# GeWu-Lab/Crab

Measured on AMD Instinct MI355X. Metric: clips/sec prefill+decode (AVQA 10s clip, 8 frames, 256 out tok), higher is better.
Workload: dtype bf16

## Files before the change

### crab_amd/_lib.py

```python
from __future__ import annotations

import ctypes as C
import os
import threading

_HERE = os.path.dirname(os.path.abspath(__file__))
LIB_PATH = os.environ.get("CRAB_HIP_LIB") or os.path.join(_HERE, "libcrab_hip.so")


class CrabHipError(RuntimeError):
    pass


class GemmDesc(C.Structure):
    _fields_ = [
        ("A", C.c_void_p), ("B", C.c_void_p), ("C", C.c_void_p), ("bias", C.c_void_p), ("R", C.c_void_p),
        ("A2", C.c_void_p), ("B2", C.c_void_p),
        ("lda", C.c_int64), ("ldb", C.c_int64), ("ldc", C.c_int64), ("ldr", C.c_int64), ("lda2", C.c_int64),
        ("ldb2", C.c_int64),
        ("M", C.c_int32), ("N", C.c_int32), ("K", C.c_int32), ("K2", C.c_int32),
        ("act", C.c_int32), ("c_fp32", C.c_int32), ("res_scale", C.c_float),
        ("batch", C.c_int32), ("nb0", C.c_int32),
        ("sA0", C.c_int64), ("sA1", C.c_int64), ("sB0", C.c_int64), ("sB1", C.c_int64), ("sC0", C.c_int64),
        ("sC1", C.c_int64), ("sR0", C.c_int64), ("sR1", C.c_int64), ("sBias0", C.c_int64), ("sBias1", C.c_int64),
# ... 123 lines not shown
    "crab_trace_end": (_i64, [_vp, C.c_char_p, _i64]),
    "crab_gemm_bf16": (_i, [_vp, _vp, C.POINTER(GemmDesc)]),
    "crab_rowfin_workspace": (_i64, [_i, _i]),
    "crab_rowfin_lora_ok": (_i, [_i, _i, _i]),
    "crab_attn_decode_rope_workspace": (_i64, [_i, _i, _i]),
    "crab_attn_decode_rope": (_i, [_vp, _vp, _vp, _i64, _vp, _vp, _vp, _vp, _i64, _i, _i, _i, _i, _i, _i, _vp, _f, _vp, _i64]),
    "crab_attn_prefix_workspace": (_i64, [_i, _i, _i]),
    "crab_attn_prefix_partial": (_i, [_vp, _vp, _vp, _i64, _vp, _vp, _vp, _i64, _vp, _i, _vp, _i, _i, _i, _i, _i, _i, _i, _f]),
    "crab_attn_own_merge": (_i, [_vp, _vp, _vp, _i64, _vp, _i64, _vp, _vp, _vp, _i64, _i, _i, _i, _i, _i, _i, _i, _vp, _f, _vp]),
    "crab_hyperlora_mix": (_i, [_vp, _vp, _vp, _i64, _i, _vp, _i64, _i, _i, _i, _i, _i, _f]),
    "crab_hyperlora_route_workspace": (_i64, [_i, _i, _i]),
    "crab_hyperlora_route": (_i, [_vp, _vp, _vp, _i64, _vp, _i64, _i, _i, _i, _i, _i, _vp, _i64, _i, _f, _vp, _i64]),
    "crab_rmsnorm": (_i, [_vp, _vp, _vp, _i64, _vp, _vp, _i64, _i, _i, _f]),
    "crab_layernorm": (_i, [_vp, _vp, _vp, _i64, _vp, _vp, _vp, _i64, _i, _i, _f]),
    "crab_embedding": (_i, [_vp, _vp, _vp, _vp, _vp, _i64, _i, _i, _i]),
    "crab_embedding_f32": (_i, [_vp, _vp, _vp, _vp, _vp, _i64, _i, _i, _i]),
    "crab_rmsnorm_f32": (_i, [_vp, _vp, _vp, _i64, _vp, _vp, _i64, _i, _i, _f]),
    "crab_layernorm_f32": (_i, [_vp, _vp, _vp, _i64, _vp, _vp, _vp, _i64, _i, _i, _f]),
    "crab_rmsnorm_p": (_i, [_vp, _vp, _vp, _i, _i64, _vp, _i, _vp, _i64, _i, _i, _f]),
    "crab_layernorm_p": (_i, [_vp, _vp, _vp, _i, _i64, _vp, _vp, _i, _vp, _i64, _i, _i, _f]),
    "crab_clip_embed_ln_p": (_i, [_vp, _vp, _vp, _vp, _vp, _vp, _vp, _i, _vp, _i, _i, _i, _f]),
    "crab_cast_rows_bf16_f32": (_i, [_vp, _vp, _vp, _i64, _vp, _i64, _i, _i]),
    "crab_cast_rows_f32_bf16": (_i, [_vp, _vp, _vp, _i64, _vp, _i64, _i, _i]),
    "crab_rope_table": (_i, [_vp, _vp, _vp, _i, _i, _f]),
    "crab_qkv_rope_split": (_i, [_vp, _vp, _vp, _i64, _vp, _vp, _vp, _vp, _i64, _i, _i, _i, _i, _i, _i, _i, _vp]),
    "crab_qkv_rope_split_ids": (_i, [_vp, _vp, _vp, _i64, _vp, _vp, _vp, _vp, _i64, _i, _i, _i, _i, _i, _i, _i, _vp, _vp, _i64]),
    "crab_qkv_rope_split_ragged": (_i, [_vp, _vp, _vp, _i64, _vp, _vp, _vp, _vp, _i64, _i, _i, _i, _i, _i, _i, _i, _vp, _vp]),
    "crab_kv_quant_fp8": (_i, [_vp, _vp, _vp, _vp, _i64, _i, _i, _vp, _vp, _i64, _vp, _vp, _i64, _i, _i, _i, _i, _i, _i, _i, _i, _vp]),
    "crab_weight_quant_fp8": (_i, [_vp, _vp, _vp, _i64, _i, _i, _vp, _i64, _vp]),
    "crab_attn_decode_fp8": (_i, [_vp, _vp, _vp, _i64, _vp, _vp, _vp, _vp, _vp, _vp, _i64, _i, _i, _i, _i, _i, _i, _vp, _f, _vp]),
    "crab_attn_decode_masked": (_i, [_vp, _vp, _vp, _i64, _vp, _vp, _vp, _i64, _i, _i, _i, _i, _i, _i, _vp, _f, _vp]),
    "crab_attn_decode_keymask": (_i, [_vp, _vp, _vp, _i64, _vp, _vp, _vp, _i64, _i, _i, _i, _i, _i, _i, _vp, _f, _vp, _i64]),
    "crab_attn_fwd": (_i, [_vp, _vp, C.POINTER(AttnDesc)]),
    "crab_attn_decode": (_i, [_vp, _vp, _vp, _i64, _vp, _vp, _vp, _i64, _i, _i, _i, _i, _i, _i, _vp, _f]),
    "crab_swiglu": (_i, [_vp, _vp, _vp, _i64, _vp, _i64, _i, _i]),
    "crab_argmax": (_i, [_vp, _vp, _vp, _i64, _vp, _i, _i, _i]),
    "crab_im2col_patch": (_i, [_vp, _vp, _vp, _i, _vp, _i64, _i, _i, _i, _i, _i]),
    "crab_clip_embed_ln": (_i, [_vp, _vp, _vp, _vp, _vp, _vp, _vp, _vp, _i, _i, _i, _f]),
    "crab_beats_posconv_pad": (_i, [_vp, _vp, _vp, _vp, _i, _i, _i, _i, _i]),
    "crab_beats_relpos_bias": (_i, [_vp, _vp, _vp, _vp, _i, _i, _i, _i]),
    "crab_beats_gru_gate": (_i, [_vp, _vp, _vp, _i64, _vp, _vp, _vp, _vp, _i, _i, _i, _i]),
    "crab_copy_rows": (_i, [_vp, _vp, _vp, _i64, _vp, _i64, _i, _i]),
    "crab_cast_f32_bf16": (_i, [_vp, _vp, _vp, _vp, _i64]),
    "crab_copy_rows_batched": (_i, [_vp, _vp, _vp, _i64, _i64, _vp, _i64, _i64, _i, _i, _i]),
    "crab_greedy_select": (_i, [_vp, _vp, _vp, _i64, _i, _i, _vp, _vp, _i64, _vp, _vp, _i, _i, _i]),
    "crab_advance": (_i, [_vp, _vp, _vp, _vp]),
    "crab_sample_select": (_i, [_vp, _vp, _vp, _i64, _i, _i, _vp, _vp, _i64, _vp, _vp, _i, _i, _i, _f, _i, _f, C.c_uint64]),
    "crab_constrained_select": (_i, [_vp, _vp, _vp, _i64, _i, _i, _vp, _vp, _vp, _i, _i, _vp, _vp, _vp, _i64, _vp, _vp, _i, _i, _i, _f, _i, _f,
                                     C.c_uint64]),
    "crab_logprob_norm": (_i, [_vp, _vp, _vp, _i64, _i, _i, _vp, _vp, _i, _i, _vp, _vp, _vp, _i, _i, _vp]),
    "crab_logprob_gather": (_i, [_vp, _vp, _vp, _i64, _i, _i, _vp, _vp, _vp, _vp, _i64, _i64, _i]),
    "crab_logits_edit": (_i, [_vp, _vp, _vp, _i64, _i, _i, _vp, _i64, _i, _vp, _vp, _f, _i, _vp, _i, _i, _vp, _vp, _i64]),
    "crab_logits_restore": (_i, [_vp, _vp, _vp, _i64, _i, _i, _vp, _vp, _vp, _i, _vp, _vp, _i64, _i]),
    "crab_lm_head_xent_workspace": (_i64, [_i, _i]),
    "crab_lm_head_xent": (_i, [_vp, _vp, _vp, _i64, _vp, _i, _vp, _i64, _i, _i, _vp, _vp, _vp, _vp, _vp, _i64]),
    "crab_xent_reduce": (_i, [_vp, _vp, _vp, _vp, _vp, _vp, _i, _vp, _vp, _vp, _vp]),
    "crab_im2col3x3": (_i, [_vp, _vp, _vp, _vp, _i, _i, _i, _i]),
    "crab_pixel_shuffle2x": (_i, [_vp, _vp, _vp, _vp, _vp, _i, _i, _i]),
    "crab_bilinear": (_i, [_vp, _vp, _vp, _i, _i64, _i64, _i64, _i, _i, _i, _vp, _i, _i, _f, _f]),
    "crab_dense_pe": (_i, [_vp, _vp, _vp, _vp, _i, _i, _i]),
    "crab_add_rows": (_i, [_vp, _vp, _vp, _i64, _vp, _i64, _i, _vp, _i64, _i, _i]),
    "crab_mask_gate": (_i, [_vp, _vp, _vp, _i64, _i, _vp, _i64, _i, _i]),
    "crab_act_inplace": (_i, [_vp, _vp, _vp, _i64, _i]),
    "crab_dist_unique_id": (_i, [_vp, _vp]),
    "crab_dist_init": (_i, [_vp, _vp, _i, _i, C.POINTER(_vp)]),
    "crab_gather_results": (_i, [_vp, _vp, _vp, _vp, _i64, _vp, _i]),
# ... 87 lines not shown
```

### crab_amd/csrc/attn.hip

```cpp
#include "common.h"
#include "crab_internal.h"
#include "attn_decode_core.h"
#include <math.h>
#include <stdlib.h>

namespace {

struct AttnP {
    const bf16_t* q; const bf16_t* k; const bf16_t* vt; bf16_t* o;
    long q_bs, q_hs, q_ss, k_bs, k_hs, k_ss, vt_bs, vt_hs, vt_ds, o_bs, o_ss;
    const float* bias; const float* gate;
    const int* kv_start;
    const uint32_t* key_mask; long key_mask_ld;
    int B, H, Hk, Sq, Skv, causal;
    float scale;
};

constexpr int KT = 64;
constexpr int VT_LD = 68;

template <int HD>
__device__ __forceinline__ int k_swz(int row, int chunk) {
    return HD == 128 ? (chunk ^ (row & 15)) : (HD == 64 ? (chunk ^ ((row >> 1) & 7)) : (chunk ^ ((0x78 >> (((row >> 2) & 3) * 2)) & 3)));
}
// ... 159 lines not shown
        for (int kk = 0; kk < 2; ++kk) {
            union { bf16x8_t v; uint32_t w[4]; } pf;
            pf.w[0] = pack_bf2(s[2 * kk][0], s[2 * kk][1]);
            pf.w[1] = pack_bf2(s[2 * kk][2], s[2 * kk][3]);
            pf.w[2] = pack_bf2(s[2 * kk + 1][0], s[2 * kk + 1][1]);
            pf.w[3] = pack_bf2(s[2 * kk + 1][2], s[2 * kk + 1][3]);
#pragma unroll
            for (int dt = 0; dt < DT; ++dt) {
                const bf16_t* vr = lv + (dt * 16 + fr) * VT_LD + kk * 32 + fg * 4;
                union { bf16x8_t v; u32x2 h[2]; } vf;
                vf.h[0] = *reinterpret_cast<const u32x2*>(vr);
                vf.h[1] = *reinterpret_cast<const u32x2*>(vr + 16);
                oacc[dt] = __builtin_amdgcn_mfma_f32_16x16x32_bf16(vf.v, pf.v, oacc[dt], 0, 0, 0);
            }
        }
    }
    l_run += __shfl_xor(l_run, 16, 64);
    l_run += __shfl_xor(l_run, 32, 64);
    const float inv = l_run > 0.f ? 1.0f / l_run : 0.f;
    if (qrow < p.Sq) {
        bf16_t* op = p.o + (long)b * p.o_bs + (long)qrow * p.o_ss + (long)h * HD;
#pragma unroll
        for (int dt = 0; dt < DT; ++dt) {
            u32x2 w;
            w[0] = pack_bf2(oacc[dt][0] * inv, oacc[dt][1] * inv);
            w[1] = pack_bf2(oacc[dt][2] * inv, oacc[dt][3] * inv);
            *reinterpret_cast<u32x2*>(op + dt * 16 + fg * 4) = w;
        }
    }
}


typedef __attribute__((ext_vector_type(16))) float f32x16_t;

template <int HD, bool CAUSAL>
__global__ __launch_bounds__(256, 2) void attn_fwd32_kernel(AttnP p) {
    constexpr int CPR = HD / 8;
    constexpr int KS = HD / 16;
    constexpr int DT = HD / 32;
    constexpr int KBUF = KT * HD, VBUF = HD * VT_LD;
    __shared__ __attribute__((aligned(16))) bf16_t lk[2 * KBUF];
    __shared__ __attribute__((aligned(16))) bf16_t lv[2 * VBUF];

    const int tid = threadIdx.x, lane = tid & 63;
    const int wave = __builtin_amdgcn_readfirstlane(tid >> 6);
    const int fc = lane & 31, fg = lane >> 5;
    const int nqb = (p.Sq + 127) >> 7;
    const int lid = xcd_remap(blockIdx.x, gridDim.x);
    const int b = lid / (nqb * p.H), h = (lid / nqb) % p.H;
    const int hk = h / (p.H / p.Hk);
    const int q0 = (nqb - 1 - lid % nqb) * 128;
    const int qw0 = q0 + wave * 32;
    const int qrow = qw0 + fc;
    const int qload = qrow < p.Sq ? qrow : p.Sq - 1;
    const int koff = p.Skv - p.Sq;
    const bool wave_on = qw0 < p.Sq;

    const bf16_t* qp = p.q + (long)b * p.q_bs + (long)h * p.q_hs + (long)qload * p.q_ss;
    const bf16_t* kp = p.k + (long)b * p.k_bs + (long)hk * p.k_hs;
    const bf16_t* vp = p.vt + (long)b * p.vt_bs + (long)hk * p.vt_hs;

    bf16x8_t qf[KS];
#pragma unroll
    for (int ks = 0; ks < KS; ++ks) qf[ks] = *reinterpret_cast<const bf16x8_t*>(qp + ks * 16 + fg * 8);

    f32x16_t oacc[DT];
// ... 98 lines not shown
                for (int r = 0; r < 16; ++r) {
                    const float e = __builtin_amdgcn_exp2f(__builtin_fmaf(s[j][r], sc2, -m_new));
                    s[j][r] = e;
                    psum += e;
                }
            l_run = l_run * alpha + psum;
            if (__any(raised)) {
#pragma unroll
                for (int i = 0; i < DT; ++i) oacc[i] *= alpha;
            }
#pragma unroll
            for (int j = 0; j < 2; ++j)
#pragma unroll
                for (int kk = 0; kk < 2; ++kk) {
                    union { bf16x8_t v; uint32_t w[4]; } pf;
                    pf.w[0] = pack_bf2(s[j][8 * kk + 0], s[j][8 * kk + 1]);
                    pf.w[1] = pack_bf2(s[j][8 * kk + 2], s[j][8 * kk + 3]);
                    pf.w[2] = pack_bf2(s[j][8 * kk + 4], s[j][8 * kk + 5]);
                    pf.w[3] = pack_bf2(s[j][8 * kk + 6], s[j][8 * kk + 7]);
#pragma unroll
                    for (int dt = 0; dt < DT; ++dt) {
                        const bf16_t* vr = lvc + (dt * 32 + fc) * VT_LD + j * 32 + kk * 16 + fg * 4;
                        union { bf16x8_t v; u32x2 hh[2]; } vf;
                        vf.hh[0] = *reinterpret_cast<const u32x2*>(vr);
                        vf.hh[1] = *reinterpret_cast<const u32x2*>(vr + 8);
                        oacc[dt] = __builtin_amdgcn_mfma_f32_32x32x16_bf16(vf.v, pf.v, oacc[dt], 0, 0, 0);
                    }
                }
        }
        __syncthreads();
    }
    l_run += __shfl_xor(l_run, 32, 64);
    const float inv = l_run > 0.f ? 1.0f / l_run : 0.f;
    if (qrow < p.Sq) {
        bf16_t* op = p.o + (long)b * p.o_bs + (long)qrow * p.o_ss + (long)h * HD;
#pragma unroll
        for (int dt = 0; dt < DT; ++dt)
#pragma unroll
            for (int g4 = 0; g4 < 4; ++g4) {
                u32x2 w;
                w[0] = pack_bf2(oacc[dt][4 * g4 + 0] * inv, oacc[dt][4 * g4 + 1] * inv);
                w[1] = pack_bf2(oacc[dt][4 * g4 + 2] * inv, oacc[dt][4 * g4 + 3] * inv);
                *reinterpret_cast<u32x2*>(op + dt * 32 + g4 * 8 + fg * 4) = w;
            }
    }
}
#undef ATT_LOAD_TILE
#undef ATT_MASK_V
#undef ATT_STORE_TILE

template <int HD>
__global__ __launch_bounds__(256) void attn_decode_kernel(const bf16_t* __restrict__ q, long ldq, const bf16_t* __restrict__ kc,
                                                          const bf16_t* __restrict__ vc, bf16_t* __restrict__ o, long ldo, int H, int Hk,
                                                          int Tmax, int ctx_host, const int* __restrict__ ctx_dev, float scale,
                                                          const int* __restrict__ kv_start) {
    constexpr int EPL = HD / 16;
    const int tid = threadIdx.x;
    const int grp = tid >> 4, sub = tid & 15;
    const int b = blockIdx.y, h = blockIdx.x;
    const int hk = h / (H / Hk);
    const int ks0 = kv_start ? kv_start[b] : 0;
    const int ctx = ctx_host + (ctx_dev ? ctx_dev[0] : 0) - ks0;
    const bf16_t* qp = q + (long)b * ldq + (long)h * HD + sub * EPL;
    float qv[EPL];
#pragma unroll
    for (int e = 0; e < EPL; ++e) qv[e] = bf2f(qp[e]) * scale;
    const bf16_t* kb = kc + (((long)b * Hk + hk) * (long)Tmax + ks0) * HD + sub * EPL;
    const bf16_t* vb = vc + (((long)b * Hk + hk) * (long)Tmax + ks0) * HD + sub * EPL;
    float m = -1e30f, l = 0.f, acc[EPL];
#pragma unroll
    for (int e = 0; e < EPL; ++e) acc[e] = 0.f;
    if constexpr (EPL == 8) {
        dec_stream(qv, kb, vb, ctx, grp, m, l, acc);
    } else {
        for (int j = grp; j < ctx; j += 16) {
            float kx[EPL], vx[EPL];
            const u32x2 kw = __builtin_nontemporal_load(reinterpret_cast<const u32x2*>(kb + (long)j * HD));
            const u32x2 vw = __builtin_nontemporal_load(reinterpret_cast<const u32x2*>(vb + (long)j * HD));
#pragma unroll
            for (int e = 0; e < 2; ++e) { kx[2 * e] = lo_bf(kw[e]); kx[2 * e + 1] = hi_bf(kw[e]); vx[2 * e] = lo_bf(vw[e]); vx[2 * e + 1] = hi_bf(vw[e]); }
            float sdot = 0.f;
#pragma unroll
// ... 382 lines not shown
#pragma unroll
                for (int g = 0; g < G; ++g) {
                    const float pg = g < 4 ? p0[g & 3] : p1[g & 3];
#pragma unroll
                    for (int e = 0; e < EPL; ++e) acc[g][e] += pg * vx[e];
                }
            }
        }
    }
    __syncthreads();
#pragma unroll
    for (int g = 0; g < G; ++g)
#pragma unroll
        for (int e = 0; e < EPL; ++e) {
            float v = acc[g][e];
            v += __shfl_xor(v, 16, 64);
            v += __shfl_xor(v, 32, 64);
            acc[g][e] = v;
        }
    if (lane < 16) {
#pragma unroll
        for (int g = 0; g < G; ++g)
#pragma unroll
            for (int e = 0; e < EPL; ++e) sbuf[(wave * G + g) * HD + sub * EPL + e] = acc[g][e];
    }
    __syncthreads();
    for (int idx = tid; idx < G * HD; idx += 256) {
        const float O = (sbuf[idx] + sbuf[G * HD + idx]) + (sbuf[2 * G * HD + idx] + sbuf[3 * G * HD + idx]);
        const int g = idx / HD;
        o[(long)b * ldo + (long)(hk * G) * HD + idx] = f2bf(O / l_run[g]);
    }
}

}

extern "C" int crab_attn_fwd(crab_ctx* ctx, void* stream, const crab_attn_desc* d) {
    if (!ctx) return CRAB_E_INVALID;
    if (!d || !d->q || !d->k || !d->vt || !d->o) return crab_fail(ctx, CRAB_E_INVALID, "attn_fwd: null operand");
    if (d->B <= 0 || d->H <= 0 || d->Hk <= 0 || d->H % d->Hk || d->Sq <= 0 || d->Skv <= 0)
        return crab_fail(ctx, CRAB_E_INVALID, "attn_fwd: bad shape");
    if (d->head_dim != 32 && d->head_dim != 64 && d->head_dim != 128) return crab_fail(ctx, CRAB_E_UNSUPPORTED, "attn_fwd: head_dim must be 32, 64 or 128");
    if (d->head_dim == 32 && (d->causal || d->bias)) return crab_fail(ctx, CRAB_E_UNSUPPORTED, "attn_fwd: head_dim 32 only without mask/bias");
    if ((d->q_ss & 7) || (d->q_hs & 7) || (d->q_bs & 7) || (d->k_ss & 7) || (d->k_hs & 7) || (d->k_bs & 7) || (d->vt_ds & 7) ||
        (d->vt_hs & 7) || (d->vt_bs & 7) || (d->o_ss & 3) || (d->o_bs & 3))
        return crab_fail(ctx, CRAB_E_INVALID, "attn_fwd: strides must keep 16-byte alignment");
    if (((uintptr_t)d->q & 15) || ((uintptr_t)d->k & 15) || ((uintptr_t)d->vt & 15) || ((uintptr_t)d->o & 7))
        return crab_fail(ctx, CRAB_E_INVALID, "attn_fwd: pointer alignment");
    if (d->causal && d->Skv < d->Sq) return crab_fail(ctx, CRAB_E_INVALID, "attn_fwd: causal needs Skv >= Sq");
    if ((d->bias == nullptr) && d->gate) return crab_fail(ctx, CRAB_E_INVALID, "attn_fwd: gate without bias");
    if (d->key_mask && (d->key_mask_ld < (d->Skv + 31) / 32 || d->head_dim == 32))
        return crab_fail(ctx, CRAB_E_INVALID, "attn_fwd: key_mask needs key_mask_ld >= ceil(Skv / 32) words per sequence (head_dim 64 / 128)");
    AttnP p;
    p.q = (const bf16_t*)d->q; p.k = (const bf16_t*)d->k; p.vt = (const bf16_t*)d->vt; p.o = (bf16_t*)d->o;
    p.q_bs = d->q_bs; p.q_hs = d->q_hs; p.q_ss = d->q_ss; p.k_bs = d->k_bs; p.k_hs = d->k_hs; p.k_ss = d->k_ss;
    p.vt_bs = d->vt_bs; p.vt_hs = d->vt_hs; p.vt_ds = d->vt_ds; p.o_bs = d->o_bs; p.o_ss = d->o_ss;
    p.bias = d->bias; p.gate = d->gate; p.kv_start = d->kv_start; p.key_mask = d->key_mask; p.key_mask_ld = d->key_mask_ld; p.B = d->B; p.H = d->H; p.Hk = d->Hk; p.Sq = d->Sq; p.Skv = d->Skv;
    p.causal = d->causal; p.scale = d->scale;
    dim3 grid(((d->Sq + 63) / 64) * d->H * d->B), block(256);
    hipStream_t s = (hipStream_t)stream;
    const bool hb = d->bias != nullptr;
    if (d->causal && hb) return crab_fail(ctx, CRAB_E_UNSUPPORTED, "attn_fwd: causal + bias not instantiated");
    static const int fwd32 = []() { const char* e = getenv("CRAB_ATTN_FWD32"); return !(e && e[0] == '0'); }();
    if (fwd32 && !hb && d->Sq > 64 && d->scale > 0.f && (d->head_dim == 128 || d->head_dim == 64)) {
        dim3 grid32(((d->Sq + 127) / 128) * d->H * d->B);
        if (d->head_dim == 128) {
            if (d->causal) hipLaunchKernelGGL((attn_fwd32_kernel<128, true>), grid32, block, 0, s, p);
            else hipLaunchKernelGGL((attn_fwd32_kernel<128, false>), grid32, block, 0, s, p);
        } else {
            if (d->causal) hipLaunchKernelGGL((attn_fwd32_kernel<64, true>), grid32, block, 0, s, p);
            else hipLaunchKernelGGL((attn_fwd32_kernel<64, false>), grid32, block, 0, s, p);
        }
        return crab_check_launch(ctx, d->head_dim == 128 ? (d->causal ? "attn_fwd32_kernel<128,causal>" : "attn_fwd32_kernel<128>")
                                                         : (d->causal ? "attn_fwd32_kernel<64,causal>" : "attn_fwd32_kernel<64>"));
    }
    if (d->head_dim == 32) {
        hipLaunchKernelGGL((attn_fwd_kernel<32, false, false>), grid, block, 0, s, p);
    } else if (d->head_dim == 128) {
        if (d->causal) hipLaunchKernelGGL((attn_fwd_kernel<128, true, false>), grid, block, 0, s, p);
        else if (hb) hipLaunchKernelGGL((attn_fwd_kernel<128, false, true>), grid, block, 0, s, p);
        else hipLaunchKernelGGL((attn_fwd_kernel<128, false, false>), grid, block, 0, s, p);
    } else {
        if (d->causal) hipLaunchKernelGGL((attn_fwd_kernel<64, true, false>), grid, block, 0, s, p);
        else if (hb) hipLaunchKernelGGL((attn_fwd_kernel<64, false, true>), grid, block, 0, s, p);
        else hipLaunchKernelGGL((attn_fwd_kernel<64, false, false>), grid, block, 0, s, p);
    }
    return crab_check_launch(ctx, d->head_dim == 32 ? "attn_fwd_kernel<32>" : d->head_dim == 128 ? (d->causal ? "attn_fwd_kernel<128,causal>" : hb ? "attn_fwd_kernel<128,bias>" : "attn_fwd_kernel<128>")
                                                                            : (d->causal ? "attn_fwd_kernel<64,causal>" : hb ? "attn_fwd_kernel<64,bias>" : "attn_fwd_kernel<64>"));
}

extern "C" int64_t crab_attn_decode_rope_workspace(int B, int H, int d) {
    return ((int64_t)B * H * 8 * (d + 2) * 4 + 255) / 256 * 256 + (int64_t)B * H * 4;
}

extern "C" int crab_attn_decode_rope(crab_ctx* ctx, void* stream, const void* qkv, int64_t ldqkv, const float* rope_tab, void* k_cache,
                                     void* v_cache, void* o, int64_t ldo, int B, int H, int Hk, int d, int Tmax, int pos0,
                                     const int32_t* pos_dev, float scale, void* workspace, int64_t workspace_bytes) {
    if (!ctx) return CRAB_E_INVALID;
    if (!qkv || !rope_tab || !k_cache || !v_cache || !o || B <= 0 || H <= 0 || Hk <= 0 || H % Hk) return crab_fail(ctx, CRAB_E_INVALID, "attn_decode_rope: bad argument");
    if (d != 64 && d != 128) return crab_fail(ctx, CRAB_E_UNSUPPORTED, "attn_decode_rope: head_dim must be 64 or 128");
    if ((ldqkv & 7) || ((uintptr_t)qkv & 15) || ((uintptr_t)k_cache & 15) || ((uintptr_t)v_cache & 15)) return crab_fail(ctx, CRAB_E_INVALID, "attn_decode_rope: alignment");
    if (!pos_dev && (pos0 < 0 || pos0 >= Tmax)) return crab_fail(ctx, CRAB_E_INVALID, "attn_decode_rope: position outside the KV cache");
    int nsplit = 1;
    static const int tgt = []() { const char* e = getenv("CRAB_ATTN_BLOCKS"); return e ? atoi(e) : 512; }();
    if ((long)B * H < tgt) { nsplit = (int)(tgt / ((long)B * H)); if (nsplit > 8) nsplit = 8; }
    if (nsplit > 1 && (!workspace || workspace_bytes < crab_attn_decode_rope_workspace(B, H, d)))
        return crab_fail(ctx, CRAB_E_WORKSPACE, "attn_decode_rope: needs crab_attn_decode_rope_workspace(B, H, d) bytes (counters zeroed once)");
    float* part = (float*)workspace;
    unsigned* counters = workspace ? (unsigned*)((char*)workspace + ((int64_t)B * H * 8 * (d + 2) * 4 + 255) / 256 * 256) : nullptr;
    hipStream_t s = (hipStream_t)stream;
    static const int wide_on = []() { const char* e = getenv("CRAB_ATTN_WIDE"); return !(e && e[0] == '0'); }();
    if (wide_on && nsplit == 2 && d == 128) {
        hipLaunchKernelGGL((attn_decode_rope_kernel<128, 32>), dim3(H, B, 1), dim3(512), 0, s, (const bf16_t*)qkv, (long)ldqkv, rope_tab, (bf16_t*)k_cache,
                           (bf16_t*)v_cache, (bf16_t*)o, (long)ldo, H, Hk, Tmax, pos0, pos_dev, scale, (float*)nullptr, (unsigned*)nullptr);
        return crab_check_launch(ctx, "attn_decode_rope_kernel<128,32>");
    }
    dim3 grid(H, B, nsplit), block(256);
    if (d == 128)
        hipLaunchKernelGGL((attn_decode_rope_kernel<128>), grid, block, 0, s, (const bf16_t*)qkv, (long)ldqkv, rope_tab, (bf16_t*)k_cache,
                           (bf16_t*)v_cache, (bf16_t*)o, (long)ldo, H, Hk, Tmax, pos0, pos_dev, scale, part, counters);
    else
// ... 59 lines not shown
```

### crab_amd/ops.py

```python
from __future__ import annotations

import ctypes as C
import os
from typing import Optional

import torch

from . import _lib
from ._lib import AttnDesc, GemmDesc

ACT = {"none": 0, None: 0, "gelu": 1, "quick_gelu": 2, "relu": 3, "silu": 4, "swiglu_pair": 5}
BF16 = torch.bfloat16


def _stream():
    return C.c_void_p(torch.cuda.current_stream().cuda_stream)


def _dev(t: torch.Tensor) -> int:
    if not t.is_cuda:
        raise _lib.CrabHipError("crab_amd ops need CUDA/HIP tensors (no CPU fallback exists)")
    return t.device.index or 0


# ... 307 lines not shown
        _lib.check(_lib.load().crab_cast_rows_f32_bf16(_lib.ctx(d), _stream(), _p(src), lds, _p(dst), dst.stride(0), rows, cols), d)
    else:
        raise _lib.CrabHipError(f"cast_rows: {src.dtype} -> {dst.dtype} is not supported")
    return dst


def rope_table(max_pos: int, head_dim: int, theta: float, device) -> torch.Tensor:
    tab = torch.empty((max_pos, head_dim // 2, 2), device=device, dtype=torch.float32)
    d = _dev(tab)
    _lib.check(_lib.load().crab_rope_table(_lib.ctx(d), _stream(), _p(tab), max_pos, head_dim, theta), d)
    return tab


def qkv_rope_split(qkv: torch.Tensor, rope_tab: Optional[torch.Tensor], k_cache: Optional[torch.Tensor],
                   v_cache: Optional[torch.Tensor], vt: Optional[torch.Tensor], B: int, S: int, H: int, Hk: int, d_: int,
                   Tmax: int, pos0: int = 0, pos_dev: Optional[torch.Tensor] = None, pos_ids: Optional[torch.Tensor] = None,
                   row_off: Optional[torch.Tensor] = None):
    d = _dev(qkv)
    vt_ld = vt.stride(-2) if vt is not None else 0
    if row_off is not None:
        if pos_ids is not None:
            raise ValueError("qkv_rope_split: pos_ids and row_off are alternatives")
        _lib.check(_lib.load().crab_qkv_rope_split_ragged(_lib.ctx(d), _stream(), _p(qkv), qkv.stride(0), _p(rope_tab), _p(k_cache), _p(v_cache),
                                                          _p(vt), vt_ld, B, S, H, Hk, d_, Tmax, pos0, _p(pos_dev), _p(row_off)), d)
        return
    if pos_ids is not None and (pos_ids.dtype != torch.int32 or pos_ids.dim() != 2 or pos_ids.stride(1) != 1):
        raise ValueError("pos_ids must be an int32 [B, S] tensor with contiguous rows")
    _lib.check(_lib.load().crab_qkv_rope_split_ids(_lib.ctx(d), _stream(), _p(qkv), qkv.stride(0), _p(rope_tab), _p(k_cache), _p(v_cache),
                                                   _p(vt), vt_ld, B, S, H, Hk, d_, Tmax, pos0, _p(pos_dev), _p(pos_ids),
                                                   pos_ids.stride(0) if pos_ids is not None else 0), d)


def attn_fwd(q, k, vt, o, *, q_strides, k_strides, vt_strides, o_strides, B, H, Hk, Sq, Skv, head_dim, scale, causal=False,
             bias=None, gate=None, kv_start=None, key_mask=None):
    d = _dev(q)
    a = AttnDesc()
    a.q, a.k, a.vt, a.o = q.data_ptr(), k.data_ptr(), vt.data_ptr(), o.data_ptr()
    a.q_bs, a.q_hs, a.q_ss = q_strides
    a.k_bs, a.k_hs, a.k_ss = k_strides
    a.vt_bs, a.vt_hs, a.vt_ds = vt_strides
    a.o_bs, a.o_ss = o_strides
    a.bias = bias.data_ptr() if bias is not None else None
    a.gate = gate.data_ptr() if gate is not None else None
    a.kv_start = kv_start.data_ptr() if kv_start is not None else None
    if key_mask is not None:
        if key_mask.dtype != torch.int32 or key_mask.dim() != 2 or key_mask.stride(1) != 1 or key_mask.shape[0] != B:
            raise ValueError("key_mask must be an int32 [B, words] tensor with contiguous rows (ops.pack_key_mask)")
        a.key_mask, a.key_mask_ld = key_mask.data_ptr(), key_mask.stride(0)
    a.B, a.H, a.Hk, a.Sq, a.Skv, a.head_dim, a.causal, a.scale = B, H, Hk, Sq, Skv, head_dim, 1 if causal else 0, scale
    _lib.check(_lib.load().crab_attn_fwd(_lib.ctx(d), _stream(), C.byref(a)), d)
    return o


def pack_key_mask(mask: torch.Tensor) -> torch.Tensor:
    m = mask.reshape(mask.shape[0], -1).ne(0)
    B, T = m.shape
    W = (T + 31) // 32
    mp = torch.zeros(B, W * 32, dtype=torch.int64, device=m.device)
    mp[:, :T] = m
    v = (mp.view(B, W, 32) << torch.arange(32, device=m.device)).sum(-1)
    return torch.where(v >= 2 ** 31, v - 2 ** 32, v).to(torch.int32).contiguous()


def attn_decode(q, k_cache, v_cache, o, B, H, Hk, head_dim, Tmax, ctx_len, scale, ctx_dev=None, kv_start=None, key_mask=None):
    d = _dev(q)
    if key_mask is not None:
        if kv_start is not None:
            raise ValueError("attn_decode: key_mask already carries the left padding, pass one of the two")
        if key_mask.dtype != torch.int32 or key_mask.dim() != 2 or key_mask.stride(1) != 1 or key_mask.shape[0] != B:
            raise ValueError("key_mask must be an int32 [B, words] tensor with contiguous rows (ops.pack_key_mask)")
        _lib.check(_lib.load().crab_attn_decode_keymask(_lib.ctx(d), _stream(), _p(q), q.stride(0), _p(k_cache), _p(v_cache), _p(o), o.stride(0),
                                                        B, H, Hk, head_dim, Tmax, ctx_len, _p(ctx_dev), scale, _p(key_mask), key_mask.stride(0)), d)
        return o
    prof = PROFILER
    sample = prof is not None and prof.decode_eager and prof.decode_ctx > 0 and not torch.cuda.is_current_stream_capturing()
    if sample:
        e0 = torch.cuda.Event(enable_timing=True); e1 = torch.cuda.Event(enable_timing=True)
        e0.record()
    _lib.check(_lib.load().crab_attn_decode_masked(_lib.ctx(d), _stream(), _p(q), q.stride(0), _p(k_cache), _p(v_cache), _p(o), o.stride(0),
                                                   B, H, Hk, head_dim, Tmax, ctx_len, _p(ctx_dev), scale, _p(kv_start)), d)
    if sample:
        e1.record()
        nbytes = 2.0 * B * prof.decode_ctx * Hk * head_dim * 2 + 2.0 * B * H * head_dim * 2
# ... 614 lines not shown
```

### include/crab_hip.h

```cpp
#ifndef CRAB_HIP_H
#define CRAB_HIP_H

#include <stdint.h>

#ifdef __cplusplus
extern "C" {
#endif

#define CRAB_OK 0
#define CRAB_E_INVALID (-1)
#define CRAB_E_HIP (-2)
#define CRAB_E_UNSUPPORTED (-3)
#define CRAB_E_WORKSPACE (-4)

typedef struct crab_ctx crab_ctx;

int crab_ctx_create(int device, crab_ctx** out);
void crab_ctx_destroy(crab_ctx* ctx);
const char* crab_last_error(crab_ctx* ctx);
int crab_sync(crab_ctx* ctx, void* stream);
int crab_abi_version(void);
int crab_trace_begin(crab_ctx* ctx);
int64_t crab_trace_end(crab_ctx* ctx, char* buf , int64_t n);
int crab_sizeof_gemm_desc(void);
// ... 61 lines not shown
int crab_rmsnorm_p(crab_ctx* ctx, void* stream, const void* x, int x_fp32, int64_t ldx, const void* w, int w_fp32, void* y, int64_t ldy,
                   int M, int D, float eps);

int crab_embedding(crab_ctx* ctx, void* stream, const int64_t* ids, const void* table, void* out, int64_t ldo,
                   int T, int D, int vocab);
int crab_embedding_f32(crab_ctx* ctx, void* stream, const int64_t* ids, const void* table, float* out, int64_t ldo,
                       int T, int D, int vocab);

int crab_rope_table(crab_ctx* ctx, void* stream, float* tab, int max_pos, int head_dim, float theta);

int crab_qkv_rope_split(crab_ctx* ctx, void* stream, void* qkv, int64_t ldqkv, const float* rope_tab,
                        void* k_cache, void* v_cache, void* vt, int64_t vt_ld, int B, int S, int H, int Hk, int d,
                        int Tmax, int pos0, const int32_t* pos_dev);

int crab_qkv_rope_split_ids(crab_ctx* ctx, void* stream, void* qkv, int64_t ldqkv, const float* rope_tab,
                            void* k_cache, void* v_cache, void* vt, int64_t vt_ld, int B, int S, int H, int Hk, int d,
                            int Tmax, int pos0, const int32_t* pos_dev, const int32_t* pos_ids, int64_t ld_pos);

int crab_qkv_rope_split_ragged(crab_ctx* ctx, void* stream, void* qkv, int64_t ldqkv, const float* rope_tab,
                               void* k_cache, void* v_cache, void* vt, int64_t vt_ld, int B, int S, int H, int Hk, int d,
                               int Tmax, int pos0, const int32_t* pos_dev, const int32_t* row_off);


typedef struct {
    const void* q; const void* k; const void* vt; void* o;
    int64_t q_bs, q_hs, q_ss, k_bs, k_hs, k_ss, vt_bs, vt_hs, vt_ds, o_bs, o_ss;
    const float* bias; const float* gate;
    int32_t B, H, Hk, Sq, Skv, head_dim, causal;
    float scale;
    const int32_t* kv_start;
    const uint32_t* key_mask; int64_t key_mask_ld;
} crab_attn_desc;
int crab_attn_fwd(crab_ctx* ctx, void* stream, const crab_attn_desc* d);

int crab_attn_decode(crab_ctx* ctx, void* stream, const void* q, int64_t ldq, const void* k_cache, const void* v_cache,
                     void* o, int64_t ldo, int B, int H, int Hk, int d, int Tmax, int ctx_len_host,
                     const int32_t* ctx_dev, float scale);

int crab_attn_decode_masked(crab_ctx* ctx, void* stream, const void* q, int64_t ldq, const void* k_cache, const void* v_cache,
                            void* o, int64_t ldo, int B, int H, int Hk, int d, int Tmax, int ctx_len_host,
                            const int32_t* ctx_dev, float scale, const int32_t* kv_start);
int crab_attn_decode_keymask(crab_ctx* ctx, void* stream, const void* q, int64_t ldq, const void* k_cache, const void* v_cache,
                             void* o, int64_t ldo, int B, int H, int Hk, int d, int Tmax, int ctx_len_host, const int32_t* ctx_dev,
                             float scale, const uint32_t* key_mask, int64_t key_mask_ld);

#define CRAB_ATTN_SPLIT_BELOW 257
int64_t crab_attn_decode_rope_workspace(int B, int H, int d);
int crab_attn_decode_rope(crab_ctx* ctx, void* stream, const void* qkv, int64_t ldqkv, const float* rope_tab, void* k_cache,
                          void* v_cache, void* o, int64_t ldo, int B, int H, int Hk, int d, int Tmax, int pos0,
                          const int32_t* pos_dev, float scale, void* workspace, int64_t workspace_bytes);

int64_t crab_attn_prefix_workspace(int rows, int H, int d);
int crab_attn_prefix_partial(crab_ctx* ctx, void* stream, const void* q, int64_t ldq, const void* prefix_k, const void* prefix_v,
                             void* workspace, int64_t workspace_bytes, const int32_t* tile_rows, int ntiles, const int32_t* row_clip,
                             int rows, int C, int H, int Hk, int d, int Tp, int P, float scale);
int crab_attn_own_merge(crab_ctx* ctx, void* stream, const void* q, int64_t ldq, const void* workspace, int64_t workspace_bytes,
                        const void* k_cache, const void* v_cache, void* o, int64_t ldo, int B, int Sq, int H, int Hk, int d, int Tmax,
                        int ctx_len_host, const int32_t* ctx_dev, float scale, const int32_t* kv_start);

int crab_kv_quant_fp8(crab_ctx* ctx, void* stream, const void* k_src, const void* v_src, int64_t src_layer_stride, int T_src, int t0,
                      void* k_codes, void* v_codes, int64_t code_layer_stride, float* k_scale, float* v_scale,
                      int64_t scale_layer_stride, int L, int Bc, int Hk, int d, int Tmax, int b0, int t_dst, int S,
                      const int32_t* row_off);
int crab_attn_decode_fp8(crab_ctx* ctx, void* stream, const void* qkv, int64_t ldqkv, const float* rope_tab, void* k_codes,
                         void* v_codes, float* k_scale, float* v_scale, void* o, int64_t ldo, int B, int H, int Hk, int d, int Tmax,
                         int pos0, const int32_t* pos_dev, float scale, const int32_t* kv_start);
// ... 189 lines not shown
```

Before: 30.96.

## Add 8-wave ping-pong attention forward kernel and wide permlane output stores

Adds an opt-in 512-thread attention prefill kernel in which two wave groups are staggered by one KV tile, so one group's QK/PV MFMA work can overlap the other's softmax and global-to-LDS loads. It is reachable only through a new form argument, since the automatic flags are off. The existing 4-wave kernel's epilogue is also changed to use permlane32 swaps, giving 16-byte output stores when the output pointer and strides are aligned. That store path runs by default and aims to cut store instruction count, at the cost of extra cross-lane swap operations.

```diff
diff --git a/crab_amd/_lib.py b/crab_amd/_lib.py
--- a/crab_amd/_lib.py
+++ b/crab_amd/_lib.py
@@ -179,6 +179,7 @@
     "crab_attn_decode_masked": (_i, [_vp, _vp, _vp, _i64, _vp, _vp, _vp, _i64, _i, _i, _i, _i, _i, _i, _vp, _f, _vp]),
     "crab_attn_decode_keymask": (_i, [_vp, _vp, _vp, _i64, _vp, _vp, _vp, _i64, _i, _i, _i, _i, _i, _i, _vp, _f, _vp, _i64]),
     "crab_attn_fwd": (_i, [_vp, _vp, C.POINTER(AttnDesc)]),
+    "crab_attn_fwd_form": (_i, [_vp, _vp, C.POINTER(AttnDesc), _i]),
     "crab_attn_decode": (_i, [_vp, _vp, _vp, _i64, _vp, _vp, _vp, _i64, _i, _i, _i, _i, _i, _i, _vp, _f]),
     "crab_swiglu": (_i, [_vp, _vp, _vp, _i64, _vp, _i64, _i, _i]),
     "crab_argmax": (_i, [_vp, _vp, _vp, _i64, _vp, _i, _i, _i]),
diff --git a/crab_amd/csrc/attn.hip b/crab_amd/csrc/attn.hip
--- a/crab_amd/csrc/attn.hip
+++ b/crab_amd/csrc/attn.hip
@@ -215,6 +215,38 @@
 
 
 typedef __attribute__((ext_vector_type(16))) float f32x16_t;
+
+template <int HD>
+__device__ __forceinline__ void fwd32_store(const AttnP& p, const f32x16_t* oacc, float inv, int b, int h, int qrow, int fg) {
+    constexpr int DT = HD / 32;
+    bf16_t* op = p.o + (long)b * p.o_bs + (long)qrow * p.o_ss + (long)h * HD;
+    const bool wide = ((reinterpret_cast<uintptr_t>(p.o) | (uintptr_t)(p.o_bs * 2) | (uintptr_t)(p.o_ss * 2)) & 15) == 0;
+    if (wide) {
+#pragma unroll
+        for (int dt = 0; dt < DT; ++dt)
+#pragma unroll
+            for (int m = 0; m < 2; ++m) {
+                uint32_t w[4];
+#pragma unroll
+                for (int i = 0; i < 4; ++i) w[i] = pack_bf2(oacc[dt][8 * m + 2 * i] * inv, oacc[dt][8 * m + 2 * i + 1] * inv);
+                const auto s0 = __builtin_amdgcn_permlane32_swap(w[0], w[2], false, false);
+                const auto s1 = __builtin_amdgcn_permlane32_swap(w[1], w[3], false, false);
+                if (qrow < p.Sq) *reinterpret_cast<u32x4*>(op + dt * 32 + m * 16 + fg * 8) = u32x4{s0[0], s1[0], s0[1], s1[1]};
+            }
+        return;
+    }
+    if (qrow < p.Sq) {
+#pragma unroll
+        for (int dt = 0; dt < DT; ++dt)
+#pragma unroll
+            for (int g4 = 0; g4 < 4; ++g4) {
+                u32x2 w;
+                w[0] = pack_bf2(oacc[dt][4 * g4 + 0] * inv, oacc[dt][4 * g4 + 1] * inv);
+                w[1] = pack_bf2(oacc[dt][4 * g4 + 2] * inv, oacc[dt][4 * g4 + 3] * inv);
+                *reinterpret_cast<u32x2*>(op + dt * 32 + g4 * 8 + fg * 4) = w;
+            }
+    }
+}
 
 template <int HD, bool CAUSAL>
 __global__ __launch_bounds__(256, 2) void attn_fwd32_kernel(AttnP p) {
@@ -379,22 +411,254 @@
     }
     l_run += __shfl_xor(l_run, 32, 64);
     const float inv = l_run > 0.f ? 1.0f / l_run : 0.f;
-    if (qrow < p.Sq) {
-        bf16_t* op = p.o + (long)b * p.o_bs + (long)qrow * p.o_ss + (long)h * HD;
-#pragma unroll
-        for (int dt = 0; dt < DT; ++dt)
-#pragma unroll
-            for (int g4 = 0; g4 < 4; ++g4) {
-                u32x2 w;
-                w[0] = pack_bf2(oacc[dt][4 * g4 + 0] * inv, oacc[dt][4 * g4 + 1] * inv);
-                w[1] = pack_bf2(oacc[dt][4 * g4 + 2] * inv, oacc[dt][4 * g4 + 3] * inv);
-                *reinterpret_cast<u32x2*>(op + dt * 32 + g4 * 8 + fg * 4) = w;
-            }
-    }
+    fwd32_store<HD>(p, oacc, inv, b, h, qrow, fg);
 }
 #undef ATT_LOAD_TILE
 #undef ATT_MASK_V
 #undef ATT_STORE_TILE
+
+template <int HD, bool CAUSAL>
+__global__ __launch_bounds__(512) void attn_fwd32pp_kernel(AttnP p) {
+    constexpr int CPR = HD / 8;
+    constexpr int KS = HD / 16;
+    constexpr int DT = HD / 32;
+    constexpr int KBUF = KT * HD, VBUF = HD * VT_LD;
+    __shared__ __attribute__((aligned(16))) bf16_t lk[2 * KBUF];
+    __shared__ __attribute__((aligned(16))) bf16_t lv[2 * VBUF];
+
+    const int tid = threadIdx.x, lane = tid & 63;
+    const int wave = __builtin_amdgcn_readfirstlane(tid >> 6);
+    const int grp = wave >> 2;
+    const int fc = lane & 31, fg = lane >> 5;
+    const int nqb = (p.Sq + 255) >> 8;
+    const int lid = xcd_remap(blockIdx.x, gridDim.x);
+    const int b = lid / (nqb * p.H), h = (lid / nqb) % p.H;
+    const int hk = h / (p.H / p.Hk);
+    const int q0 = (nqb - 1 - lid % nqb) * 256;
+    const int qw0 = q0 + wave * 32;
+    const int qrow = qw0 + fc;
+    const int qload = qrow < p.Sq ? qrow : p.Sq - 1;
+    const int koff = p.Skv - p.Sq;
+    const bool wave_on = qw0 < p.Sq;
+
+    const bf16_t* qp = p.q + (long)b * p.q_bs + (long)h * p.q_hs + (long)qload * p.q_ss;
+    const bf16_t* kp = p.k + (long)b * p.k_bs + (long)hk * p.k_hs;
+    const bf16_t* vp = p.vt + (long)b * p.vt_bs + (long)hk * p.vt_hs;
+
+    bf16x8_t qf[KS];
+#pragma unroll
+    for (int ks = 0; ks < KS; ++ks) qf[ks] = *reinterpret_cast<const bf16x8_t*>(qp + ks * 16 + fg * 8);
+
+    f32x16_t oacc[DT];
+#pragma unroll
+    for (int i = 0; i < DT; ++i)
+#pragma unroll
+        for (int r = 0; r < 16; ++r) oacc[i][r] = 0.f;
+    float m_run = -1e30f, l_run = 0.f;
+
+    int kv_end = p.Skv;
+    if (CAUSAL) kv_end = min(kv_end, q0 + 256 + koff);
+    const int ntiles = (kv_end + KT - 1) / KT;
+    const int ks0 = p.kv_start ? p.kv_start[b] : 0;
+    const int t0 = ks0 / KT;
+    const uint32_t* km = p.key_mask ? p.key_mask + (long)b * p.key_mask_ld : nullptr;
+    constexpr int NKV = (KT * CPR) / 512, NVV = (HD * 8) / 512;
+    u32x4 kreg[NKV], vreg[NVV];
+#define PP_LOAD_K(T_)                                                                                          \
+    {                                                                                                          \
+        const int kvl_ = (T_) * KT;                                                                            \
+        _Pragma("unroll") for (int i = 0; i < NKV; ++i) {                                                      \
+            const int idx = tid + i * 512;                                                                     \
+            const int row = idx / CPR, c = idx % CPR;                                                          \
+            const int kr = min(kvl_ + row, p.Skv - 1);                                                         \
+            kreg[i] = *reinterpret_cast<const u32x4*>(kp + (long)kr * p.k_ss + c * 8);                         \
+        }                                                                                                      \
+    }
+#define PP_LOAD_V(T_)                                                                                          \
+    {                                                                                                          \
+        const int kvl_ = (T_) * KT;                                                                            \
+        _Pragma("unroll") for (int i = 0; i < NVV; ++i) {                                                      \
+            const int idx = tid + i * 512;                                                                     \
+            const int row = idx >> 3, c = idx & 7;                                                             \
+            int kc = kvl_ + c * 8;                          \
+            kc = kc < p.Skv ? kc : 0;                                                                          \
+            vreg[i] = *reinterpret_cast<const u32x4*>(vp + (long)row * p.vt_ds + kc);                          \
+        }                                                                                                      \
+    }
+#define PP_STORE_K(T_)                                                                                         \
+    {                                                                                                          \
+        bf16_t* lk_ = lk + ((T_) & 1) * KBUF;                                                                  \
+        _Pragma("unroll") for (int i = 0; i < NKV; ++i) {                                                      \
+            const int idx = tid + i * 512;                                                                     \
+            const int row = idx / CPR, c = idx % CPR;                                                          \
+            *reinterpret_cast<u32x4*>(lk_ + row * HD + (k_swz<HD>(row, c) << 3)) = kreg[i];                    \
+        }                                                                                                      \
+    }
+#define PP_STORE_V(T_)                                                                                         \
+    {                                                                                                          \
+        if ((T_) * KT + KT > p.Skv) {                                                                          \
+            _Pragma("unroll") for (int i = 0; i < NVV; ++i) {                                                  \
+                const int c = (tid + i * 512) & 7;                                                             \
+                const int rem = p.Skv - ((T_) * KT + c * 8);     \
+                _Pragma("unroll") for (int w = 0; w < 4; ++w) {                                                \
+                    const uint32_t m = (2 * w < rem ? 0x0000ffffu : 0u) | (2 * w + 1 < rem ? 0xffff0000u : 0u); \
+                    vreg[i][w] &= m;                                                                           \
+                }                                                                                              \
+            }                                                                                                  \
+        }                                                                                                      \
+        bf16_t* lv_ = lv + ((T_) & 1) * VBUF;                                                                  \
+        _Pragma("unroll") for (int i = 0; i < NVV; ++i) {                                                      \
+            const int idx = tid + i * 512;                                                                     \
+            const int row = idx >> 3, c = idx & 7;                                                             \
+            bf16_t* d_ = lv_ + row * VT_LD + c * 8;                                                            \
+            *reinterpret_cast<u32x2*>(d_) = u32x2{vreg[i][0], vreg[i][1]};                                     \
+            *reinterpret_cast<u32x2*>(d_ + 4) = u32x2{vreg[i][2], vreg[i][3]};                                 \
+        }                                                                                                      \
+    }
+#define PP_PV(B_)                                                                                              \
+    {                                                                                                          \
+        const bf16_t* lvc = lv + (B_) * VBUF;                                                                  \
+        _Pragma("unroll") for (int j = 0; j < 2; ++j)                                                          \
+        _Pragma("unroll") for (int kk = 0; kk < 2; ++kk)                                                       \
+        _Pragma("unroll") for (int dt = 0; dt < DT; ++dt) {                                                    \
+            const bf16_t* vr = lvc + (dt * 32 + fc) * VT_LD + j * 32 + kk * 16 + fg * 4;                       \
+            union { bf16x8_t v; u32x2 hh[2]; } vf;                                                             \
+            vf.hh[0] = *reinterpret_cast<const u32x2*>(vr);                                                    \
+            vf.hh[1] = *reinterpret_cast<const u32x2*>(vr + 8);                                                \
+            oacc[dt] = __builtin_amdgcn_mfma_f32_32x32x16_bf16(vf.v, pfr[j * 2 + kk], oacc[dt], 0, 0, 0);      \
+        }                                                                                                      \
+    }
+#define PP_BARRIER()                                                                                           \
+    {                                                                                                          \
+        __builtin_amdgcn_sched_barrier(0);                                                                     \
+        __builtin_amdgcn_s_barrier();                                                                          \
+        __builtin_amdgcn_sched_barrier(0);                                                                     \
+    }
+    if (t0 >= ntiles) {
+        if (qrow < p.Sq) {
+            bf16_t* op = p.o + (long)b * p.o_bs + (long)qrow * p.o_ss + (long)h * HD;
+#pragma unroll
+            for (int c = 0; c < HD / 4; ++c) *reinterpret_cast<u32x2*>(op + c * 4 + 0) = u32x2{0u, 0u};
+        }
+        return;
+    }
+    PP_LOAD_K(t0)
+    if (grp == 1) PP_LOAD_V(t0)
+    PP_STORE_K(t0)
+    if (grp == 1) {
+        PP_STORE_V(t0)
+        if (t0 + 1 < ntiles) {
+            PP_LOAD_K(t0 + 1)
+            PP_STORE_K(t0 + 1)
+        }
+    }
+    if (t0 + 1 + grp < ntiles) PP_LOAD_K(t0 + 1 + grp)
+    if (t0 + grp < ntiles) PP_LOAD_V(t0 + grp)
+    asm volatile("s_waitcnt lgkmcnt(0)" ::: "memory");
+    PP_BARRIER()
+    const float sc2 = p.scale * 1.4426950408889634f;
+    bf16x8_t pfr[4];
+    bool prev_live = false;
+    if (grp == 1) PP_BARRIER()
+    for (int t = t0; t < ntiles; ++t) {
+        const int kv0 = t * KT;
+        const bool live = wave_on && !(CAUSAL && kv0 > qw0 + 31 + koff);
+        f32x16_t s[2];
+        __builtin_amdgcn_s_setprio(1);
+        if (prev_live) PP_PV((t - 1) & 1)
+        if (live) {
+            const bf16_t* lkc = lk + (t & 1) * KBUF;
+#pragma unroll
+            for (int j = 0; j < 2; ++j)
+#pragma unroll
+                for (int r = 0; r < 16; ++r) s[j][r] = 0.f;
+#pragma unroll
+            for (int ks = 0; ks < KS; ++ks) {
+#pragma unroll
+                for (int j = 0; j < 2; ++j) {
+                    const int row = j * 32 + fc;
+                    const int chunk = ks * 2 + fg;
+                    bf16x8_t kf = *reinterpret_cast<const bf16x8_t*>(lkc + row * HD + (k_swz<HD>(row, chunk) << 3));
+                    s[j] = __builtin_amdgcn_mfma_f32_32x32x16_bf16(kf, qf[ks], s[j], 0, 0, 0);
+                }
+            }
+        }
+        __builtin_amdgcn_s_setprio(0);
+        PP_BARRIER()
+        if (t + 1 + grp < ntiles) PP_STORE_K(t + 1 + grp)
+        if (t + grp < ntiles) PP_STORE_V(t + grp)
+        if (t + 2 + grp < ntiles) PP_LOAD_K(t + 2 + grp)
+        if (t + 1 + grp < ntiles) PP_LOAD_V(t + 1 + grp)
+        if (live) {
+            const bool need_mask = (kv0 + KT > p.Skv) || (CAUSAL && (kv0 + KT - 1 > qw0 + koff)) || (kv0 < ks0) || km;
+            if (need_mask) {
+#pragma unroll
+                for (int j = 0; j < 2; ++j)
+#pragma unroll
+                    for (int r = 0; r < 16; ++r) {
+                        const int kv = kv0 + j * 32 + (r >> 2) * 8 + fg * 4 + (r & 3);
+                        bool ok = kv < p.Skv && kv >= ks0;
+                        if (CAUSAL) ok = ok && (kv <= qrow + koff);
+                        if (km) ok = ok && ((km[min(kv, p.Skv - 1) >> 5] >> (kv & 31)) & 1u);
+                        s[j][r] = ok ? s[j][r] : -INFINITY;
+                    }
+            }
+            float tmax = -INFINITY;
+#pragma unroll
+            for (int j = 0; j < 2; ++j)
+#pragma unroll
+                for (int r = 0; r < 16; r += 2) tmax = fmaxf(tmax, fmaxf(s[j][r], s[j][r + 1]));
+            tmax = fmaxf(tmax, __shfl_xor(tmax, 32, 64));
+            const float m_new = fmaxf(m_run, tmax * sc2);
+            const float alpha = __builtin_amdgcn_exp2f(m_run - m_new);
+            const bool raised = m_new != m_run;
+            m_run = m_new;
+            float psum = 0.f;
+#pragma unroll
+            for (int j = 0; j < 2; ++j)
+#pragma unroll
+                for (int r = 0; r < 16; ++r) {
+                    const float e = __builtin_amdgcn_exp2f(__builtin_fmaf(s[j][r], sc2, -m_new));
+                    s[j][r] = e;
+                    psum += e;
+                }
+            l_run = l_run * alpha + psum;
+            if (__any(raised)) {
+#pragma unroll
+                for (int i = 0; i < DT; ++i) oacc[i] *= alpha;
+            }
+#pragma unroll
+            for (int j = 0; j < 2; ++j)
+#pragma unroll
+                for (int kk = 0; kk < 2; ++kk) {
+                    union { bf16x8_t v; uint32_t w[4]; } pf;
+                    pf.w[0] = pack_bf2(s[j][8 * kk + 0], s[j][8 * kk + 1]);
+                    pf.w[1] = pack_bf2(s[j][8 * kk + 2], s[j][8 * kk + 3]);
+                    pf.w[2] = pack_bf2(s[j][8 * kk + 4], s[j][8 * kk + 5]);
+                    pf.w[3] = pack_bf2(s[j][8 * kk + 6], s[j][8 * kk + 7]);
+                    pfr[j * 2 + kk] = pf.v;
+                }
+        }
+        prev_live = live;
+        asm volatile("s_waitcnt lgkmcnt(0)" ::: "memory");
+        PP_BARRIER()
+    }
+    if (prev_live) {
+        __builtin_amdgcn_s_setprio(1);
+        PP_PV((ntiles - 1) & 1)
+        __builtin_amdgcn_s_setprio(0);
+    }
+    if (grp == 0) PP_BARRIER()
+    l_run += __shfl_xor(l_run, 32, 64);
+    const float inv = l_run > 0.f ? 1.0f / l_run : 0.f;
+    fwd32_store<HD>(p, oacc, inv, b, h, qrow, fg);
+}
+#undef PP_LOAD_K
+#undef PP_LOAD_V
+#undef PP_STORE_K
+#undef PP_STORE_V
+#undef PP_PV
+#undef PP_BARRIER
 
 template <int HD>
 __global__ __launch_bounds__(256) void attn_decode_kernel(const bf16_t* __restrict__ q, long ldq, const bf16_t* __restrict__ kc,
@@ -843,9 +1107,22 @@
     }
 }
 
-}
-
-extern "C" int crab_attn_fwd(crab_ctx* ctx, void* stream, const crab_attn_desc* d) {
+constexpr bool PP_AUTO_D128 = false, PP_AUTO_D64 = false;
+
+int attn_fwd_dispatch(crab_ctx* ctx, void* stream, const crab_attn_desc* d, int form);
+
+}
+
+extern "C" int crab_attn_fwd(crab_ctx* ctx, void* stream, const crab_attn_desc* d) { return attn_fwd_dispatch(ctx, stream, d, 0); }
+
+extern "C" int crab_attn_fwd_form(crab_ctx* ctx, void* stream, const crab_attn_desc* d, int form) {
+    if (!ctx) return CRAB_E_INVALID;
+    if (form < 0 || form > 2) return crab_fail(ctx, CRAB_E_INVALID, "attn_fwd_form: form must be 0 (automatic), 1 (4 waves) or 2 (8 waves)");
+    return attn_fwd_dispatch(ctx, stream, d, form);
+}
+
+namespace {
+int attn_fwd_dispatch(crab_ctx* ctx, void* stream, const crab_attn_desc* d, int form) {
     if (!ctx) return CRAB_E_INVALID;
     if (!d || !d->q || !d->k || !d->vt || !d->o) return crab_fail(ctx, CRAB_E_INVALID, "attn_fwd: null operand");
     if (d->B <= 0 || d->H <= 0 || d->Hk <= 0 || d->H % d->Hk || d->Sq <= 0 || d->Skv <= 0)
@@ -873,6 +1150,22 @@
     if (d->causal && hb) return crab_fail(ctx, CRAB_E_UNSUPPORTED, "attn_fwd: causal + bias not instantiated");
     static const int fwd32 = []() { const char* e = getenv("CRAB_ATTN_FWD32"); return !(e && e[0] == '0'); }();
     if (fwd32 && !hb && d->Sq > 64 && d->scale > 0.f && (d->head_dim == 128 || d->head_dim == 64)) {
+        const bool pp = d->Sq > 128 && (form == 2 || (form == 0 && (d->head_dim == 128 ? PP_AUTO_D128 : PP_AUTO_D64)));
+        if (pp) {
+            dim3 gridpp(((d->Sq + 255) / 256) * d->H * d->B), blockpp(512);
+            if (d->head_dim == 128) {
+                if (d->causal) hipLaunchKernelGGL((attn_fwd32pp_kernel<128, true>), gridpp, blockpp, 0, s, p);
+                else hipLaunchKernelGGL((attn_fwd32pp_kernel<128, false>), gridpp, blockpp, 0, s, p);
+            } else {
+                if (d->causal) hipLaunchKernelGGL((attn_fwd32pp_kernel<64, true>), gridpp, blockpp, 0, s, p);
+                else hipLaunchKernelGGL((attn_fwd32pp_kernel<64, false>), gridpp, blockpp, 0, s, p);
+            }
+            if (form == 2)
+                return crab_check_launch(ctx, d->head_dim == 128 ? (d->causal ? "attn_fwd32pp_kernel<128,causal>" : "attn_fwd32pp_kernel<128>")
+                                                                 : (d->causal ? "attn_fwd32pp_kernel<64,causal>" : "attn_fwd32pp_kernel<64>"));
+            return crab_check_launch(ctx, d->head_dim == 128 ? (d->causal ? "attn_fwd32_kernel<128,causal>" : "attn_fwd32_kernel<128>")
+                                                             : (d->causal ? "attn_fwd32_kernel<64,causal>" : "attn_fwd32_kernel<64>"));
+        }
         dim3 grid32(((d->Sq + 127) / 128) * d->H * d->B);
         if (d->head_dim == 128) {
             if (d->causal) hipLaunchKernelGGL((attn_fwd32_kernel<128, true>), grid32, block, 0, s, p);
@@ -897,6 +1190,7 @@
     }
     return crab_check_launch(ctx, d->head_dim == 32 ? "attn_fwd_kernel<32>" : d->head_dim == 128 ? (d->causal ? "attn_fwd_kernel<128,causal>" : hb ? "attn_fwd_kernel<128,bias>" : "attn_fwd_kernel<128>")
                                                                             : (d->causal ? "attn_fwd_kernel<64,causal>" : hb ? "attn_fwd_kernel<64,bias>" : "attn_fwd_kernel<64>"));
+}
 }
 
 extern "C" int64_t crab_attn_decode_rope_workspace(int B, int H, int d) {
diff --git a/crab_amd/ops.py b/crab_amd/ops.py
--- a/crab_amd/ops.py
+++ b/crab_amd/ops.py
@@ -363,7 +363,7 @@
 
 
 def attn_fwd(q, k, vt, o, *, q_strides, k_strides, vt_strides, o_strides, B, H, Hk, Sq, Skv, head_dim, scale, causal=False,
-             bias=None, gate=None, kv_start=None, key_mask=None):
+             bias=None, gate=None, kv_start=None, key_mask=None, form: int = 0):
     d = _dev(q)
     a = AttnDesc()
     a.q, a.k, a.vt, a.o = q.data_ptr(), k.data_ptr(), vt.data_ptr(), o.data_ptr()
@@ -379,7 +379,10 @@
             raise ValueError("key_mask must be an int32 [B, words] tensor with contiguous rows (ops.pack_key_mask)")
         a.key_mask, a.key_mask_ld = key_mask.data_ptr(), key_mask.stride(0)
     a.B, a.H, a.Hk, a.Sq, a.Skv, a.head_dim, a.causal, a.scale = B, H, Hk, Sq, Skv, head_dim, 1 if causal else 0, scale
-    _lib.check(_lib.load().crab_attn_fwd(_lib.ctx(d), _stream(), C.byref(a)), d)
+    if form:
+        _lib.check(_lib.load().crab_attn_fwd_form(_lib.ctx(d), _stream(), C.byref(a), form), d)
+    else:
+        _lib.check(_lib.load().crab_attn_fwd(_lib.ctx(d), _stream(), C.byref(a)), d)
     return o
 
 
diff --git a/include/crab_hip.h b/include/crab_hip.h
--- a/include/crab_hip.h
+++ b/include/crab_hip.h
@@ -117,6 +117,7 @@
     const uint32_t* key_mask; int64_t key_mask_ld;
 } crab_attn_desc;
 int crab_attn_fwd(crab_ctx* ctx, void* stream, const crab_attn_desc* d);
+int crab_attn_fwd_form(crab_ctx* ctx, void* stream, const crab_attn_desc* d, int form);
 
 int crab_attn_decode(crab_ctx* ctx, void* stream, const void* q, int64_t ldq, const void* k_cache, const void* v_cache,
                      void* o, int64_t ldo, int B, int H, int Hk, int d, int Tmax, int ctx_len_host,
```

Measured after the change: 30.95. About the same (-0.0%).
